# DecodeGenetics/BamQC

Measured on AMD Instinct MI355X. Metric: BAM records/sec (and GB/s vs HBM roofline), 150 bp PE, 1/2/4/8 MI355X, higher is better.
Workload: dtype u8/u32/u64 integer

## Files before the change

bamqc_amd/csrc/k_prep.hip:

```cpp
#include <algorithm>
#include <vector>
#include "kernels_common.h"
#include "prep.h"

#define PR_THREADS 256
#define PR_PER_THREAD 4
#define PR_BLOCK (PR_THREADS * PR_PER_THREAD)

__device__ __forceinline__ uint32_t wave_scan_incl_max(uint32_t v)
{
    v = max(v, (uint32_t)__builtin_amdgcn_update_dpp(0, (int)v, 0x111, 0xF, 0xF, true));
    v = max(v, (uint32_t)__builtin_amdgcn_update_dpp(0, (int)v, 0x112, 0xF, 0xF, true));
    v = max(v, (uint32_t)__builtin_amdgcn_update_dpp(0, (int)v, 0x114, 0xF, 0xF, true));
    v = max(v, (uint32_t)__builtin_amdgcn_update_dpp(0, (int)v, 0x118, 0xF, 0xF, true));
    v = max(v, (uint32_t)__builtin_amdgcn_update_dpp(0, (int)v, 0x142, 0xA, 0xF, false));
    v = max(v, (uint32_t)__builtin_amdgcn_update_dpp(0, (int)v, 0x143, 0xC, 0xF, false));
    return v;
}
__device__ __forceinline__ uint32_t block_scan_excl(uint32_t v, uint32_t* sh, uint32_t* total)
{
    const uint32_t inc = wave_scan_incl(v), w = threadIdx.x >> 6, nw = blockDim.x >> 6;
    block_sync();
    if (lane_id() == WAVE - 1) sh[w] = inc;
    block_sync();
    uint32_t base = 0, tot = 0;
    for (uint32_t k = 0; k < nw; ++k) { const uint32_t x = sh[k]; if (k < w) base += x; tot += x; }
    *total = tot;
    return base + inc - v;
}
__device__ __forceinline__ uint32_t block_scan_excl_max(uint32_t v, uint32_t* sh, uint32_t* total)
{
    const uint32_t inc = wave_scan_incl_max(v), w = threadIdx.x >> 6, nw = blockDim.x >> 6;
    block_sync();
    if (lane_id() == WAVE - 1) sh[w] = inc;
    block_sync();
    uint32_t base = 0, tot = 0;
    for (uint32_t k = 0; k < nw; ++k) { const uint32_t x = sh[k]; if (k < w) base = max(base, x); tot = max(tot, x); }
    *total = tot;
    const uint32_t prev = (uint32_t)__builtin_amdgcn_update_dpp(0, (int)inc, 0x138 , 0xF, 0xF, true);
    return max(base, prev);
}
__device__ __forceinline__ unsigned long long uniform64(unsigned long long v)
{
    return (unsigned long long)__builtin_amdgcn_readfirstlane((uint32_t)v) | (unsigned long long)__builtin_amdgcn_readfirstlane((uint32_t)(v >> 32)) << 32;
}
__device__ __forceinline__ void err_key(ErrRec* e, uint32_t read, uint32_t order)
{
    atomicMin(&e->first_key, ((unsigned long long)read << 3) | order);
}

#define PS_THREADS 1024
#define PS_PER (PR_GROUP / (PS_THREADS / 64))
__global__ __launch_bounds__(PS_THREADS) void k_prep_sizes(PrepArgs a)
{
    __shared__ unsigned long long sh[3 * PR_GROUP];
    if (blockIdx.x == 0 && threadIdx.x == 0) {
        a.err->first_key = BQC_ERRKEY_NONE; a.err->flags = 0; a.err->aux0 = a.err->aux1 = 0;
        a.desc->n_cov_extra = 0;
        if (a.pend_extra_n) *a.pend_extra_n = 0;
        if (a.replay) *a.cursor = *a.cursor_save; else *a.cursor_save = *a.cursor;
    }
    for (uint32_t k = blockIdx.x * PS_THREADS + threadIdx.x; k < a.n_sw; k += gridDim.x * PS_THREADS) a.sw_counts[k] = SwCounts{0, 0, 0, 0};
    const uint32_t nblk = (a.n + PR_BLOCK - 1) / PR_BLOCK, bg0 = blockIdx.x * PR_GROUP, nb = min((uint32_t)PR_GROUP, nblk - bg0);
    const uint32_t w = threadIdx.x >> 6, l = lane_id();
    uint4 vl[PS_PER][4];
    uint2 vc[PS_PER][4];
#pragma unroll
    for (int q = 0; q < PS_PER; ++q) {
        const uint32_t bl = w + (PS_THREADS / 64) * q;
        const unsigned long long i0 = (unsigned long long)(bg0 + bl) * PR_BLOCK;
        const bool whole = bl < nb && i0 + PR_BLOCK <= a.n;
#pragma unroll
        for (int j = 0; j < 4; ++j) {
            vl[q][j] = make_uint4(0, 0, 0, 0); vc[q][j] = make_uint2(0, 0);
            if (whole) { const uint32_t i = (uint32_t)i0 + 256u * j + 4u * l; vl[q][j] = *(const uint4*)(a.l_seq + i); vc[q][j] = *(const uint2*)(a.n_cigar + i); }
        }
    }
#pragma unroll
    for (int q = 0; q < PS_PER; ++q) {
        const uint32_t bl = w + (PS_THREADS / 64) * q;
        const unsigned long long i0 = (unsigned long long)(bg0 + bl) * PR_BLOCK;
        unsigned long long s1 = 0, s2 = 0, s3 = 0;
#pragma unroll
        for (int j = 0; j < 4; ++j) {
            const uint4 v = vl[q][j];
            s1 += (unsigned long long)((v.x + 1) / 2) + (v.y + 1) / 2 + (v.z + 1) / 2 + (v.w + 1) / 2;
            s2 += (unsigned long long)v.x + v.y + v.z + v.w;
            s3 += (vc[q][j].x & 0xFFFFu) + (vc[q][j].x >> 16) + (vc[q][j].y & 0xFFFFu) + (vc[q][j].y >> 16);
        }
        if (bl < nb && i0 + PR_BLOCK > a.n)
            for (unsigned long long i = i0 + l; i < a.n; i += WAVE) { const uint32_t L = a.l_seq[i]; s1 += (L + 1) / 2; s2 += L; s3 += a.n_cigar[i]; }
#pragma unroll
        for (int o = 32; o > 0; o >>= 1) { s1 += __shfl_xor(s1, o); s2 += __shfl_xor(s2, o); s3 += __shfl_xor(s3, o); }
        if (l == 0) { sh[3 * bl] = s1; sh[3 * bl + 1] = s2; sh[3 * bl + 2] = s3; }
    }
    block_sync();
    if (threadIdx.x < 3 * PR_GROUP) {
        const uint32_t bl = threadIdx.x / 3, k = threadIdx.x % 3;
        unsigned long long t = 0;
        for (uint32_t j = 0; j < bl; ++j) t += sh[3 * j + k];
        if (bl < nb) a.blk_sizes[3ull * (bg0 + bl) + k] = t;
        if (bl == PR_GROUP - 1) a.grp_sizes[3ull * blockIdx.x + k] = t + sh[3 * bl + k];
    }
}

struct CigarView {
    uint32_t w[4];
    const uint32_t* cg;
    __device__ __forceinline__ uint32_t at(uint32_t k) const
    {
        if (k < 4u) return k == 0u ? w[0] : k == 1u ? w[1] : k == 2u ? w[2] : w[3];
        return cg[k];
    }
};
__device__ __forceinline__ int triplet_eligible(uint32_t flag, uint32_t mapq, int32_t as, const CigarView& cv, uint32_t ncig)
{
    if (!(flag & 0x1) || !(flag & 0x2) || (flag & 0x4) || (flag & 0x8) || (flag & 0x100)) return 0;
    if (mapq < 60) return 0;
    if (as == BQC_AS_ABSENT || as < 0) return -1;
    if (as < 50) return 0;
    uint32_t clipped = 0;
    for (uint32_t k = 0; k < ncig; ++k) {
        const uint32_t wd = cv.at(k), op = wd & 15u;
        if (op == 4u || op == 5u) clipped += wd >> 4;
    }
    return clipped > 0 ? 0 : 1;
}

struct ReadIn { uint32_t L, nc, flag, lane, mapq; int32_t rid, pos, as; CovEntry ce; };
struct ReadOut { uint32_t flag, cls, tgt1; CovEntry ce; };
__device__ __forceinline__ ReadOut prep_one(const PrepArgs& a, const DevRefs& refs, uint32_t i, const ReadIn& in, uint32_t co, bool offsets_ok,
                                            const CigarView& cv, bool ref_loaded , int32_t target_in )
{
    ReadOut o;
    uint32_t flag = in.flag & (0x0FFFu | BQC_FLAG_MATE_MAIN | BQC_FLAG_NO_QUAL);
    const uint32_t L = in.L, lane = in.lane;
    uint32_t nc = in.nc;
    o.tgt1 = 0;
    if (L > a.max_read_len) err_key(a.err, i, 1);
    else if (lane >= a.n_lanes) err_key(a.err, i, 2);
    if (!offsets_ok) nc = 0;
    const bool fast = !a.no_fast && L <= BQC_FAST_MAXLEN;
    uint32_t nseg = 0;
    CovEntry ce = in.ce;
    if (!(flag & 0x900u)) {
        const bool dup = flag & 0x400u, qcf = flag & 0x200u;
        if (!dup && !qcf) {
            const int e = triplet_eligible(flag, in.mapq, in.as, cv, nc);
            if (e < 0) err_key(a.err, i, 4);
            if (e > 0) {
                const int32_t target = target_in;
                if (target < 0 || !ref_loaded) err_key(a.err, i, 5);
                else { o.tgt1 = (uint32_t)target + 1u; flag |= BQC_FLAG_TRIPLET; }
            }
        }
        if (!(flag & 0xC0u)) err_key(a.err, i, 6);
    }
    if (ce.win != BQC_COV_NONE) {
        flag |= BQC_FLAG_COV;
        const bool rc = flag & 0x10u;
        const bool pending = ce.win == BQC_COV_PENDING;
        const uint32_t pend_idx = ce.off_len;
        const int64_t pos = pending ? 0 : (int64_t)ce.off_len;
        uint32_t cc = 0;
        int64_t run_a = -1, run_z = -1;
        bool first = true;
        ce.off_len = 0;
        auto emit = [&](int64_t lo, int64_t hi) {
            if (pending) {
                if (lo < 0 || lo >= 2 * BQC_VSIZE || lo >= hi) return;
                const uint32_t len = (uint32_t)(hi - lo < 2 * BQC_VSIZE ? hi - lo : 2 * BQC_VSIZE);
                if (first) { a.pend[pend_idx] = PendRun{(uint32_t)lo, len}; first = false; return; }
                const uint32_t k = atomicAdd(a.pend_extra_n, 1u);
                if (k < a.pend_extra_cap) a.pend_extra[k] = PendExtra{pend_idx, (uint32_t)lo, len, 0};
                else atomicOr(&a.err->flags, BQC_DEVERR_INTERNAL);
                return;
            }
            hi = hi < 2 * BQC_VSIZE ? hi : 2 * BQC_VSIZE;
            if (lo < 0 || lo >= hi) return;
            const uint32_t v = (uint32_t)lo | ((uint32_t)(hi - lo) << 16);
            if (first) { ce.off_len = v; first = false; return; }
            const uint32_t k = atomicAdd(&a.desc->n_cov_extra, 1u);
            if (k < a.cov_extra_cap) a.cov_extra[k] = CovExtra{ce.win, v, lane, 0};
            else atomicOr(&a.err->flags, BQC_DEVERR_INTERNAL);
        };
        if (nc == 1u) {
            const uint32_t w = cv.w[0], op = w & 15u, nn = w >> 4;
            if (op == 0u || op == 2u) emit(pos, pos + nn);
        } else {
            for (uint32_t k = 0; k < nc; ++k) {
                const uint32_t w = cv.at(rc ? nc - 1 - k : k), op = w & 15u, nn = w >> 4;
                if (op == 4u) cc += nn;
                if (op == 0u || op == 2u) {
                    const int64_t lo = pos + (int64_t)cc, hi = lo + nn;
                    if (run_z == lo) run_z = hi;
                    else { if (run_a >= 0) emit(run_a, run_z); run_a = lo; run_z = hi; }
                    cc += nn;
                }
            }
            if (run_a >= 0) emit(run_a, run_z);
        }
        if (pending) { if (first) a.pend[pend_idx] = PendRun{0, 0}; ce = CovEntry{BQC_COV_NONE, 0}; }
    } else ce.off_len = 0;
    if (fast && (flag & BQC_FLAG_TRIPLET) && nc > 1 && L >= 3) {
        const uint32_t n0 = cv.w[0] >> 4;
        if (n0 != 0) {
            uint64_t rp = n0;
            int64_t cpos = (int64_t)in.pos + n0;
            for (uint32_t k2 = 1; k2 < nc && rp < L; ++k2) {
                const uint32_t wk = cv.at(k2), op = wk & 15u, nn = wk >> 4;
                if (op == 2u || op == 3u || op == 5u || op == 6u) cpos += nn;
                else if (op == 4u || op == 1u) rp += nn;
                else {
                    const uint64_t ia = rp > 1 ? rp : 1, ib = rp + nn < (uint64_t)L - 1 ? rp + nn : (uint64_t)L - 1;
                    const int64_t posv = cpos - (int64_t)rp;
                    if (ia < ib && posv > INT32_MIN / 2 && posv < INT32_MAX / 2) {
                        a.segs[co + nseg] = TripSeg{i, (int32_t)posv, (uint32_t)ia | ((uint32_t)ib << 8), 0};
                        ++nseg;
                    }
                    rp += nn; cpos += nn;
                }
            }
        }
    }
    o.flag = flag;
    o.ce = ce;
    o.cls = ((fast ? ((flag & 0x40u) ? 0u : 1u) : 2u) << 8) | nseg;
    return o;
}

#ifndef PR_WAVES_PER_EU
#define PR_WAVES_PER_EU 4
#endif
__global__ __launch_bounds__(PR_THREADS) __attribute__((amdgpu_waves_per_eu(PR_WAVES_PER_EU, PR_WAVES_PER_EU))) void k_prep_reads(PrepArgs a, DevRefs refs)
{
    __shared__ uint32_t sh[2 * (PR_THREADS / 64)];
    __shared__ uint32_t red[8];
    __shared__ unsigned long long gsum[3 * (PR_THREADS / 64) + 6];
    const uint32_t i0 = blockIdx.x * PR_BLOCK + 4u * threadIdx.x;
    if (threadIdx.x < 8) red[threadIdx.x] = threadIdx.x == 0 ? 0xFFFFFFFFu : 0u;
    const uint32_t grp = blockIdx.x / PR_GROUP, nblk = gridDim.x;
    unsigned long long grp_before[3] = {0, 0, 0}, grp_more[3] = {0, 0, 0}, in_grp = 0;
    for (uint32_t g = threadIdx.x + 2 * PR_THREADS; g < grp; g += PR_THREADS) {
        const unsigned long long* p = (const unsigned long long*)((const char*)a.grp_sizes + 24u * g);
        for (int k = 0; k < 3; ++k) grp_before[k] += p[k];
    }
    if (threadIdx.x < grp) {
        const unsigned long long* p = (const unsigned long long*)((const char*)a.grp_sizes + 24u * threadIdx.x);
        for (int k = 0; k < 3; ++k) grp_before[k] += p[k];
    }
    if (threadIdx.x + PR_THREADS < grp) {
        const unsigned long long* p = (const unsigned long long*)((const char*)a.grp_sizes + 24u * (threadIdx.x + PR_THREADS));
        for (int k = 0; k < 3; ++k) grp_more[k] = p[k];
    }
    if (threadIdx.x < 6) {
        const bool grp_last = (blockIdx.x + 1) % PR_GROUP == 0 || blockIdx.x + 1 == nblk;
        const unsigned long long* incl_p = grp_last ? a.grp_sizes + 3ull * grp : a.blk_sizes + 3ull * (blockIdx.x + 1);
        in_grp = threadIdx.x < 3 ? a.blk_sizes[3ull * blockIdx.x + threadIdx.x] : incl_p[threadIdx.x - 3];
    }
    auto sum_groups = [&] {
        for (int k = 0; k < 3; ++k) grp_before[k] += grp_more[k];
#pragma unroll
        for (int o = 32; o > 0; o >>= 1)
            for (int k = 0; k < 3; ++k) grp_before[k] += __shfl_xor(grp_before[k], o);
        if (lane_id() == 0) for (int k = 0; k < 3; ++k) gsum[3 * (threadIdx.x >> 6) + k] = grp_before[k];
        if (threadIdx.x < 6) gsum[3 * (PR_THREADS / 64) + threadIdx.x] = in_grp;
    };
    ReadIn in[4];
    const uint32_t nlive = i0 >= a.n ? 0u : min(4u, a.n - i0);
    if ((unsigned long long)(blockIdx.x + 1) * PR_BLOCK <= a.n) {
        const uint4 vl = *(const uint4*)(a.l_seq + i0);
        const uint2 vc = *(const uint2*)(a.n_cigar + i0), vf = *(const uint2*)(a.flag_in + i0);
        const uint32_t vlane = *(const uint32_t*)(a.lane + i0), vmq = *(const uint32_t*)(a.mapq + i0);
        const int4 vr = *(const int4*)(a.rid + i0), vp = *(const int4*)(a.pos + i0), va = *(const int4*)(a.as_ + i0);
        const uint4 c01 = *(const uint4*)(a.cov_in + i0), c23 = *(const uint4*)(a.cov_in + i0 + 2);
        asm volatile("" : "+v"(grp_before[0]), "+v"(grp_before[1]), "+v"(grp_before[2]));
        sum_groups();
        const uint32_t Ls[4] = {vl.x, vl.y, vl.z, vl.w}, ncs[4] = {vc.x & 0xFFFFu, vc.x >> 16, vc.y & 0xFFFFu, vc.y >> 16};
        const uint32_t fs[4] = {vf.x & 0xFFFFu, vf.x >> 16, vf.y & 0xFFFFu, vf.y >> 16};
        const int32_t rs[4] = {vr.x, vr.y, vr.z, vr.w}, ps[4] = {vp.x, vp.y, vp.z, vp.w}, as[4] = {va.x, va.y, va.z, va.w};
        const CovEntry cs[4] = {{c01.x, c01.y}, {c01.z, c01.w}, {c23.x, c23.y}, {c23.z, c23.w}};
#pragma unroll
        for (int j = 0; j < 4; ++j) in[j] = ReadIn{Ls[j], ncs[j], fs[j], (vlane >> (8 * j)) & 0xFFu, (vmq >> (8 * j)) & 0xFFu, rs[j], ps[j], as[j], cs[j]};
    } else {
        sum_groups();
#pragma unroll
        for (int j = 0; j < 4; ++j) {
            in[j] = ReadIn{0, 0, 0x900u, 0, 0, -1, 0, 0, CovEntry{BQC_COV_NONE, 0}};
            if ((uint32_t)j < nlive) { const uint32_t i = i0 + j; in[j] = ReadIn{a.l_seq[i], a.n_cigar[i], a.flag_in[i], a.lane[i], a.mapq[i], a.rid[i], a.pos[i], a.as_[i], a.cov_in[i]}; }
        }
    }
    uint32_t ls[4], lq[4], lc[4], ts = 0, tq = 0, tc = 0;
#pragma unroll
    for (int j = 0; j < 4; ++j) { ls[j] = ts; lq[j] = tq; lc[j] = tc; ts += (in[j].L + 1) / 2; tq += in[j].L; tc += in[j].nc; }
    uint32_t tot;
    const uint32_t xs = block_scan_excl(ts, sh, &tot), xq = block_scan_excl(tq, sh, &tot), xc = block_scan_excl(tc, sh, &tot);
    unsigned long long excl[3], incl[3];
    for (int k = 0; k < 3; ++k) {
        unsigned long long t = 0;
        for (uint32_t w = 0; w < PR_THREADS / 64; ++w) t += gsum[3 * w + k];
        grp_before[k] = uniform64(t); excl[k] = uniform64(gsum[3 * (PR_THREADS / 64) + k]); incl[k] = uniform64(gsum[3 * (PR_THREADS / 64) + 3 + k]);
    }
    unsigned long long base[3];
    if (prep_block_bases(grp_before, excl, incl, base) && threadIdx.x == 0) err_key(a.err, blockIdx.x * PR_BLOCK, 3);
    const unsigned long long bs = base[0] + xs, bq = base[1] + xq, bc = base[2] + xc;
    ReadOut out[4];
    CigarView cv[4];
    bool ref_loaded[4];
    int32_t target[4];
    unsigned long long cos[4];
    bool oks[4];
#pragma unroll
    for (int j = 0; j < 4; ++j) {
        const unsigned long long so = bs + ls[j], qo = bq + lq[j], co = bc + lc[j];
        cos[j] = co;
        oks[j] = so + (in[j].L + 1) / 2 <= 0xFFFFFFFFull && qo + in[j].L <= 0xFFFFFFFFull && co + in[j].nc <= 0xFFFFFFFFull;
        const bool live = (uint32_t)j < nlive && oks[j];
        cv[j].cg = a.cigar + (uint32_t)co;
#pragma unroll
        for (uint32_t k = 0; k < 4u; ++k) cv[j].w[k] = live && k < in[j].nc ? cv[j].cg[k] : 0u;
        const int32_t rid = in[j].rid;
        const bool rid_ok = (uint32_t)j < nlive && rid >= 0 && (uint32_t)rid < refs.n_refs;
        ref_loaded[j] = rid_ok && refs.ref[rid] != nullptr;
        target[j] = rid_ok ? (a.fasta_index ? a.fasta_index[rid] : rid) : -1;
    }
    uint32_t tmax = 0, tmin = 0xFFFFFFFFu, maxfast = 0, maxlong = 0, cnt[4] = {0, 0, 0, 0};
    bool local_bad[4] = {false, false, false, false};
#pragma unroll
    for (int j = 0; j < 4; ++j) {
        out[j] = ReadOut{0x900u, 2u << 8, 0, CovEntry{BQC_COV_NONE, 0}};
        if ((uint32_t)j >= nlive) continue;
        out[j] = prep_one(a, refs, i0 + j, in[j], (uint32_t)cos[j], oks[j], cv[j], ref_loaded[j], target[j]);
        if (out[j].tgt1) { local_bad[j] = out[j].tgt1 < tmax; tmax = max(tmax, out[j].tgt1); tmin = min(tmin, out[j].tgt1); }
        const uint32_t cl = out[j].cls >> 8;
        if (cl == 2u) maxlong = max(maxlong, in[j].L); else maxfast = max(maxfast, in[j].L);
        cnt[cl] += 1; cnt[3] += out[j].cls & 0xFFu;
    }
    if (nlive == 4u) {
        *(uint4*)(a.seq_off + i0) = make_uint4((uint32_t)bs + ls[0], (uint32_t)bs + ls[1], (uint32_t)bs + ls[2], (uint32_t)bs + ls[3]);
        *(uint4*)(a.qual_off + i0) = make_uint4((uint32_t)bq + lq[0], (uint32_t)bq + lq[1], (uint32_t)bq + lq[2], (uint32_t)bq + lq[3]);
        *(uint4*)(a.cigar_off + i0) = make_uint4((uint32_t)bc + lc[0], (uint32_t)bc + lc[1], (uint32_t)bc + lc[2], (uint32_t)bc + lc[3]);
        *(uint2*)(a.flag_out + i0) = make_uint2(out[0].flag | (out[1].flag << 16), out[2].flag | (out[3].flag << 16));
        *(uint2*)(a.cls + i0) = make_uint2(out[0].cls | (out[1].cls << 16), out[2].cls | (out[3].cls << 16));
        *(uint4*)(a.cov_out + i0) = make_uint4(out[0].ce.win, out[0].ce.off_len, out[1].ce.win, out[1].ce.off_len);
        *(uint4*)(a.cov_out + i0 + 2) = make_uint4(out[2].ce.win, out[2].ce.off_len, out[3].ce.win, out[3].ce.off_len);
    } else {
        for (uint32_t j = 0; j < nlive; ++j) {
            const uint32_t i = i0 + j;
            a.seq_off[i] = (uint32_t)bs + ls[j]; a.qual_off[i] = (uint32_t)bq + lq[j]; a.cigar_off[i] = (uint32_t)bc + lc[j];
            a.flag_out[i] = (uint16_t)out[j].flag; a.cls[i] = (uint16_t)out[j].cls; a.cov_out[i] = out[j].ce;
        }
    }
    uint32_t blk_max;
    const uint32_t before = block_scan_excl_max(tmax, sh, &blk_max);
#pragma unroll
    for (int j = 0; j < 4; ++j)
        if (out[j].tgt1 && (local_bad[j] || out[j].tgt1 < before)) err_key(a.err, i0 + j, 5);
    if (tmin != 0xFFFFFFFFu) atomicMin(&red[0], tmin);
    if (maxfast) atomicMax(&red[1], maxfast);
    if (maxlong) atomicMax(&red[2], maxlong);
    if (!a.order) {
#pragma unroll
        for (int k = 0; k < 4; ++k) { const uint32_t v = wave_sum(cnt[k]); if (lane_id() == 0 && v) atomicAdd(&red[4 + k], v); }
    }
    block_sync();
    if (threadIdx.x == 0) {
        a.blk_tgt[2ull * blockIdx.x] = blk_max;
        a.blk_tgt[2ull * blockIdx.x + 1] = red[0];
        a.blk_maxfast[2ull * blockIdx.x] = red[1];
        a.blk_maxfast[2ull * blockIdx.x + 1] = red[2];
    }
    if (!a.order && threadIdx.x < 4 && red[4 + threadIdx.x])
        atomicAdd((uint32_t*)&a.sw_counts[blockIdx.x / (BQC_SW_READS / PR_BLOCK)] + threadIdx.x, red[4 + threadIdx.x]);
}

__device__ __forceinline__ uint32_t read_class(const PrepArgs& a, uint32_t r, uint32_t* nseg)
{
    const uint32_t v = a.cls[r];
    *nseg = v & 0xFFu;
    return v >> 8;
}

__global__ __launch_bounds__(PR_THREADS) void k_build_count(PrepArgs a)
{
    __shared__ uint32_t sh[4 * (PR_THREADS / 64)];
    const SuperWindow sw = a.sws[blockIdx.x];
    uint32_t c[4] = {0, 0, 0, 0};
    for (uint32_t p = threadIdx.x; p < sw.count; p += PR_THREADS) {
        const uint32_t r = a.order ? a.order[sw.begin + p] : sw.begin + p;
        uint32_t ns;
        const uint32_t cl = read_class(a, r, &ns);
        c[cl] += 1;
        c[3] += ns;
    }
    for (int k = 0; k < 4; ++k) c[k] = wave_sum(c[k]);
    if (lane_id() == 0) for (int k = 0; k < 4; ++k) sh[4 * (threadIdx.x >> 6) + k] = c[k];
    block_sync();
    if (threadIdx.x < 4) {
        uint32_t t = 0;
        for (uint32_t w = 0; w < PR_THREADS / 64; ++w) t += sh[4 * w + threadIdx.x];
        ((uint32_t*)&a.sw_counts[blockIdx.x])[threadIdx.x] = t;
    }
}

__global__ __launch_bounds__(1024) void k_build_plan(PrepArgs a)
{
    __shared__ uint32_t sh[2 * 16 + 8];
    __shared__ uint32_t s_fast_w, s_first_bad, s_gmin;
    const uint32_t nblk = (a.n + PR_BLOCK - 1) / PR_BLOCK;
    {
        uint32_t carry = (uint32_t)(*a.cursor + 1);
        uint32_t mf = 0, gmin = 0xFFFFFFFFu;
        if (threadIdx.x == 0) { s_first_bad = 0xFFFFFFFFu; s_gmin = 0xFFFFFFFFu; }
        for (uint32_t b0 = 0; b0 < nblk; b0 += blockDim.x) {
            const uint32_t b = b0 + threadIdx.x;
            const uint32_t mx = b < nblk ? a.blk_tgt[2ull * b] : 0u, mn = b < nblk ? a.blk_tgt[2ull * b + 1] : 0xFFFFFFFFu;
            if (b < nblk) mf = max(mf, a.blk_maxfast[2ull * b]);
            uint32_t tot;
            const uint32_t before = max(carry, block_scan_excl_max(mx, sh, &tot));
            gmin = min(gmin, mn);
            if (mn < before) atomicMin(&s_first_bad, b);
            carry = max(carry, tot);
        }
        if (gmin != 0xFFFFFFFFu) atomicMin(&s_gmin, gmin);
        block_sync();
        const uint32_t bad = s_first_bad;
        if (bad != 0xFFFFFFFFu) {
            uint32_t before = (uint32_t)(*a.cursor + 1);
            for (uint32_t b = threadIdx.x; b < bad; b += blockDim.x) before = max(before, a.blk_tgt[2ull * b]);
            uint32_t tot;
            (void)block_scan_excl_max(before, sh, &tot);
            for (uint32_t i = bad * PR_BLOCK + threadIdx.x; i < min(a.n, (bad + 1) * PR_BLOCK); i += blockDim.x)
                if (a.flag_out[i] & BQC_FLAG_TRIPLET) {
                    const int32_t rid = a.rid[i];
                    const uint32_t t1 = (uint32_t)(a.fasta_index ? a.fasta_index[rid] : rid) + 1u;
                    if (t1 < tot) err_key(a.err, i, 5);
                }
        }
        for (int o = 32; o > 0; o >>= 1) mf = max(mf, (uint32_t)__shfl_xor((int)mf, o));
        block_sync();
        if (lane_id() == 0) sh[threadIdx.x >> 6] = mf;
        block_sync();
        if (threadIdx.x == 0) {
            uint32_t m = 0;
            for (uint32_t w = 0; w < blockDim.x / 64; ++w) m = max(m, sh[w]);
            s_fast_w = max(1u, (m + 8 * BQC_FAST_NH - 1) / (8 * BQC_FAST_NH));
            *a.cursor = (int32_t)carry - 1;
            if (a.cursor[1] < 0 && s_gmin != 0xFFFFFFFFu) a.cursor[1] = (int32_t)s_gmin - 1;
        }
        block_sync();
    }
    const uint32_t fast_w = s_fast_w, rpw = 64u / fast_w, h0 = (rpw + 1) / 2, h1 = rpw / 2;
    const uint32_t groups_cap = BQC_FAST_WAVES * (64u / rpw);
    const uint32_t seg_cap = groups_cap * rpw;
    uint32_t run_g = 0, run_q = 0, run_s = 0;
    for (uint32_t s0 = 0; s0 < a.n_sw; s0 += blockDim.x) {
        const uint32_t s = s0 + threadIdx.x;
        uint32_t g = 0, q = 0, sl = 0;
        if (s < a.n_sw) {
            const SwCounts c = a.sw_counts[s];
            g = max((c.n0 + h0 - 1) / h0, (c.n1 + h1 - 1) / h1);
            q = c.n_seg; sl = c.n_slow;
        }
        uint32_t tg, tq, ts;
        const uint32_t eg = run_g + block_scan_excl(g, sh, &tg), eq = run_q + block_scan_excl(q, sh, &tq), es = run_s + block_scan_excl(sl, sh, &ts);
        if (s < a.n_sw) a.sw_plan[s] = SwPlan{eg, g, eq, es};
        run_g += tg; run_q += tq; run_s += ts;
    }
    __threadfence_block();
    block_sync();
    __shared__ uint32_t s_pb, s_cf, s_cs, s_g0, s_q0, s_s0, s_ng, s_nq, s_ns, s_lane, s_sw0, s_sw1, s_longest;
    if (threadIdx.x == 0) { s_pb = 0; s_cf = 0; s_cs = 0; }
    block_sync();
    for (uint32_t st = 0; st < a.n_stretch; ++st) {
        if (threadIdx.x == 0) {
            const Stretch S = a.stretches[st];
            const SwPlan p0 = a.sw_plan[S.sw_begin];
            const SwPlan pl = a.sw_plan[S.sw_end - 1];
            const SwCounts cl = a.sw_counts[S.sw_end - 1];
            s_g0 = p0.group_base; s_q0 = p0.seg_base; s_s0 = p0.slow_base;
            s_ng = pl.group_base + pl.n_groups - p0.group_base;
            s_nq = pl.seg_base + cl.n_seg - p0.seg_base;
            s_ns = pl.slow_base + cl.n_slow - p0.slow_base;
            s_lane = S.lane; s_sw0 = S.sw_begin; s_sw1 = S.sw_end;
        }
        block_sync();
        const uint32_t pb = s_pb, ng = s_ng, nq = s_nq, ns = s_ns, lane = s_lane;
        const uint32_t nq_pad = (nq + rpw - 1) / rpw * rpw;
        const uint32_t seg0 = pb + ng * rpw, slow0 = seg0 + nq_pad;
        for (uint32_t s = s_sw0 + threadIdx.x; s < s_sw1; s += blockDim.x) {
            SwPlan p = a.sw_plan[s];
            p.group_base = pb + (p.group_base - s_g0) * rpw;
            p.seg_base = seg0 + (p.seg_base - s_q0);
            p.slow_base = slow0 + (p.slow_base - s_s0);
            a.sw_plan[s] = p;
        }
        for (uint32_t k = nq + threadIdx.x; k < nq_pad; k += blockDim.x) a.perm[seg0 + k] = 0xFFFFFFFFu;
        const uint32_t n_rc = (ng + groups_cap - 1) / groups_cap, n_sc = (nq_pad + seg_cap - 1) / seg_cap, n_lc = (ns + BQC_CHUNK_READS - 1) / BQC_CHUNK_READS;
        const uint32_t cf = s_cf, cs = s_cs;
        for (uint32_t k = threadIdx.x; k < n_rc; k += blockDim.x) {
            const uint32_t g = min(groups_cap, ng - k * groups_cap);
            if (cf + k < a.chunks_fast_cap) a.chunks_fast[cf + k] = Chunk{pb + k * groups_cap * rpw, g * rpw, lane, g * rpw, 0, 0, 0, 0};
        }
        for (uint32_t k = threadIdx.x; k < n_sc; k += blockDim.x) {
            const uint32_t e = min(seg_cap, nq_pad - k * seg_cap);
            if (cf + n_rc + k < a.chunks_fast_cap) a.chunks_fast[cf + n_rc + k] = Chunk{seg0 + k * seg_cap, e, lane, 0, 0, 0, 0, 0};
        }
        for (uint32_t k = threadIdx.x; k < n_lc; k += blockDim.x) {
            const uint32_t e = min((uint32_t)BQC_CHUNK_READS, ns - k * BQC_CHUNK_READS);
            if (cs + k < a.chunks_slow_cap) a.chunks_slow[cs + k] = Chunk{slow0 + k * BQC_CHUNK_READS, e, lane, 0, 0, 0, 0, 0};
        }
        block_sync();
        if (threadIdx.x == 0) { s_pb = slow0 + ns; s_cf = cf + n_rc + n_sc; s_cs = cs + n_lc; }
        block_sync();
    }
    uint32_t longest = 0;
    for (uint32_t b = threadIdx.x; b < nblk; b += blockDim.x) longest = max(longest, a.blk_maxfast[2ull * b + 1]);
    for (int o = 32; o > 0; o >>= 1) longest = max(longest, (uint32_t)__shfl_xor((int)longest, o));
    if (threadIdx.x == 0) s_longest = 0;
    block_sync();
    if (lane_id() == 0) atomicMax(&s_longest, longest);
    block_sync();
    if (threadIdx.x == 0) {
        if (s_pb > a.perm_cap || s_cf > a.chunks_fast_cap || s_cs > a.chunks_slow_cap) atomicOr(&a.err->flags, BQC_DEVERR_INTERNAL);
        const bool fatal = a.err->first_key != BQC_ERRKEY_NONE || (a.err->flags & BQC_DEVERR_INTERNAL);
        a.desc->fatal = fatal ? 1u : 0u;
        a.desc->n_chunks_fast = fatal ? 0u : min(s_cf, a.chunks_fast_cap);
        a.desc->n_chunks_slow = fatal ? 0u : min(s_cs, a.chunks_slow_cap);
        a.desc->fast_w = fast_w;
        a.desc->n_perm = s_pb;
        a.desc->long_max_len = s_longest;
        if (a.desc->n_cov_extra > a.cov_extra_cap) a.desc->n_cov_extra = a.cov_extra_cap;
        const unsigned long long key = a.err->first_key;
        if (key != BQC_ERRKEY_NONE) {
            const uint32_t i = (uint32_t)(key >> 3), order = (uint32_t)key & 7u;
            if (i < a.n) { a.err->aux0 = order == 1 ? a.l_seq[i] : order == 2 ? a.lane[i] : (uint32_t)a.rid[i]; a.err->aux1 = a.lane[i]; }
        }
    }
}

__device__ __forceinline__ void block_scan_excl4(uint32_t v[4], uint32_t* sh, uint32_t tot[4])
{
    const uint32_t w = threadIdx.x >> 6, nw = blockDim.x >> 6;
    uint32_t inc[4];
#pragma unroll
    for (int k = 0; k < 4; ++k) inc[k] = wave_scan_incl(v[k]);
    block_sync();
    if (lane_id() == WAVE - 1) {
#pragma unroll
        for (int k = 0; k < 4; ++k) sh[4 * w + k] = inc[k];
    }
    block_sync();
#pragma unroll
    for (int k = 0; k < 4; ++k) {
        uint32_t base = 0, t = 0;
        for (uint32_t q = 0; q < nw; ++q) { const uint32_t x = sh[4 * q + k]; if (q < w) base += x; t += x; }
        tot[k] = t;
        v[k] = base + inc[k] - v[k];
    }
}

#define SC_PER (BQC_SW_READS / PR_THREADS)
#define SC_ENT (3 * BQC_SW_READS + 128)
__global__ __launch_bounds__(PR_THREADS) void k_build_scatter(PrepArgs a)
{
    __shared__ uint32_t ent[SC_ENT];
    __shared__ uint32_t sh[4 * (PR_THREADS / 64)];
    const SuperWindow sw = a.sws[blockIdx.x];
    const SwPlan pl = a.sw_plan[blockIdx.x];
    const uint32_t fast_w = a.desc->fast_w, rpw = 64u / fast_w, h0 = (rpw + 1) / 2, h1 = rpw / 2;
    const uint32_t n_ent = pl.n_groups * rpw;
    if (n_ent > SC_ENT) { if (threadIdx.x == 0) atomicOr(&a.err->flags, BQC_DEVERR_INTERNAL); return; }
    for (uint32_t k = threadIdx.x; k < n_ent; k += PR_THREADS) ent[k] = 0xFFFFFFFFu;
    uint32_t r[SC_PER], v[SC_PER];
    const uint32_t p0 = SC_PER * threadIdx.x;
    if (!a.order && p0 + SC_PER <= sw.count && ((sw.begin + p0) & 7u) == 0u) {
        const uint4 x = *(const uint4*)(a.cls + sw.begin + p0), y = *(const uint4*)(a.cls + sw.begin + p0 + 8);
        const uint32_t wd[8] = {x.x, x.y, x.z, x.w, y.x, y.y, y.z, y.w};
#pragma unroll
        for (int k = 0; k < SC_PER; ++k) { r[k] = sw.begin + p0 + k; v[k] = (wd[k >> 1] >> (16 * (k & 1))) & 0xFFFFu; }
    } else {
#pragma unroll
        for (int k = 0; k < SC_PER; ++k) { const uint32_t p = p0 + k; r[k] = p < sw.count ? (a.order ? a.order[sw.begin + p] : sw.begin + p) : 0xFFFFFFFFu; }
#pragma unroll
        for (int k = 0; k < SC_PER; ++k) v[k] = r[k] != 0xFFFFFFFFu ? a.cls[r[k]] : 3u << 8;
    }
    uint32_t c[4] = {0, 0, 0, 0};
#pragma unroll
    for (int k = 0; k < SC_PER; ++k) {
        const uint32_t cl = v[k] >> 8;
        c[0] += cl == 0u; c[1] += cl == 1u; c[2] += cl == 2u; c[3] += cl < 3u ? v[k] & 0xFFu : 0u;
    }
    uint32_t co[SC_PER];
#pragma unroll
    for (int k = 0; k < SC_PER; ++k) co[k] = (v[k] >> 8) < 3u && (v[k] & 0xFFu) ? a.cigar_off[r[k]] : 0u;
    uint32_t tot[4];
    block_scan_excl4(c, sh, tot);
    uint32_t k0 = c[0], k1 = c[1], k2 = c[2], k3 = c[3];
#pragma unroll
    for (int k = 0; k < SC_PER; ++k) {
        const uint32_t cl = v[k] >> 8, ns = v[k] & 0xFFu;
        if (cl == 0u) { ent[(k0 / h0) * rpw + k0 % h0] = r[k]; ++k0; }
        else if (cl == 1u) { ent[(k1 / h1) * rpw + h0 + k1 % h1] = r[k]; ++k1; }
        else if (cl == 2u) a.perm[pl.slow_base + k2++] = r[k];
        if (cl < 3u && ns) { for (uint32_t j = 0; j < ns; ++j) a.perm[pl.seg_base + k3 + j] = BQC_ENTRY_SEG | (co[k] + j); k3 += ns; }
    }
    block_sync();
    for (uint32_t k = threadIdx.x; k < n_ent; k += PR_THREADS) a.perm[pl.group_base + k] = ent[k];
}

extern "C" void bqc_launch_prep(const PrepArgs& a, const DevRefs& refs, hipStream_t s, hipEvent_t after_reads)
{
    if (a.n == 0) return;
    const uint32_t nblk = (a.n + PR_BLOCK - 1) / PR_BLOCK;
    hipLaunchKernelGGL(k_prep_sizes, dim3((nblk + PR_GROUP - 1) / PR_GROUP), dim3(PS_THREADS), 0, s, a);
    hipLaunchKernelGGL(k_prep_reads, dim3(nblk), dim3(PR_THREADS), 0, s, a, refs);
    if (after_reads) (void)hipEventRecord(after_reads, s);
    if (a.order) hipLaunchKernelGGL(k_build_count, dim3(a.n_sw), dim3(PR_THREADS), 0, s, a);
    hipLaunchKernelGGL(k_build_plan, dim3(1), dim3(1024), 0, s, a);
    hipLaunchKernelGGL(k_build_scatter, dim3(a.n_sw), dim3(PR_THREADS), 0, s, a);
}

extern "C" uint32_t bqc_prep_group(void) { return PR_GROUP; }
extern "C" uint32_t bqc_prep_bases(const uint64_t* blk_totals, uint32_t n_blocks, uint64_t* bases)
{
    const uint32_t n_groups = (n_blocks + PR_GROUP - 1) / PR_GROUP;
    std::vector<unsigned long long> blk(3ull * n_blocks), grp(3ull * n_groups);
    for (uint32_t g = 0; g < n_groups; ++g)
        for (int k = 0; k < 3; ++k) {
            unsigned long long t = 0;
            for (uint32_t b = g * PR_GROUP; b < std::min(n_blocks, (g + 1) * PR_GROUP); ++b) { blk[3ull * b + k] = t; t += blk_totals[3ull * b + k]; }
            grp[3ull * g + k] = t;
        }
    uint32_t first_bad = 0xFFFFFFFFu;
    for (uint32_t b = 0; b < n_blocks; ++b) {
        const uint32_t g = b / PR_GROUP;
        const bool grp_last = (b + 1) % PR_GROUP == 0 || b + 1 == n_blocks;
        const unsigned long long* incl = grp_last ? &grp[3ull * g] : &blk[3ull * (b + 1)];
        unsigned long long before[3] = {0, 0, 0}, base[3];
        for (uint32_t g2 = 0; g2 < g; ++g2)
            for (int k = 0; k < 3; ++k) before[k] += grp[3ull * g2 + k];
        if (prep_block_bases(before, &blk[3ull * b], incl, base)) first_bad = std::min(first_bad, b);
        for (int k = 0; k < 3; ++k) bases[3ull * b + k] = base[k];
    }
    return first_bad;
}

__device__ __forceinline__ uint32_t pend_interval(uint32_t pos, uint32_t c0, uint32_t len)
{
    const uint32_t lo = pos + c0;
    if (!len || lo >= 2u * BQC_VSIZE) return 0u;
    const uint32_t hi = min(lo + len, 2u * BQC_VSIZE);
    return lo | ((hi - lo) << 16);
}
__global__ __launch_bounds__(256) void k_pend_cov(uint32_t n, const CovEntry* __restrict__ cov_in, const PendRun* __restrict__ pend, const PendExtra* __restrict__ extra,
                                                     const uint32_t* __restrict__ extra_n, uint32_t extra_cap, const uint8_t* __restrict__ lane,
                                                     CovEntry* __restrict__ cov_out, CovExtra* __restrict__ cov_extra, BatchDesc* __restrict__ desc)
{
    const uint32_t ne = min(*extra_n, extra_cap);
    for (uint32_t i = blockIdx.x * blockDim.x + threadIdx.x; i < n; i += gridDim.x * blockDim.x) {
        const CovEntry ce = cov_in[i];
        const PendRun r = pend[i];
        cov_out[i] = CovEntry{ce.win, pend_interval(ce.off_len, r.c0, r.len)};
    }
    for (uint32_t e = blockIdx.x * blockDim.x + threadIdx.x; e < ne; e += gridDim.x * blockDim.x) {
        const PendExtra x = extra[e];
        const CovEntry ce = cov_in[x.idx];
        cov_extra[e] = CovExtra{ce.win, pend_interval(ce.off_len, x.c0, x.len), lane[x.idx], 0};
    }
    if (blockIdx.x == 0 && threadIdx.x == 0) { desc->n_cov_extra = ne; desc->fatal = 0; }
}
extern "C" void bqc_launch_pend_cov(uint32_t n, const CovEntry* cov_in, const PendRun* pend, const PendExtra* extra, const uint32_t* extra_n, uint32_t extra_cap,
                                    const uint8_t* lane, CovEntry* cov_out, CovExtra* cov_extra, BatchDesc* desc, hipStream_t s)
{
    if (!n) return;
    hipLaunchKernelGGL(k_pend_cov, dim3(std::min<uint32_t>((n + 255) / 256, 4096u)), dim3(256), 0, s, n, cov_in, pend, extra, extra_n, extra_cap, lane, cov_out, cov_extra, desc);
}
```

bamqc_amd/csrc/prep.h:

```cpp
#pragma once
#include <hip/hip_runtime.h>
#include <stdint.h>
#include "device_types.h"

#ifndef PR_GROUP
#define PR_GROUP 32
#endif
static_assert(PR_GROUP >= 16 && (PR_GROUP & (PR_GROUP - 1)) == 0, "PR_GROUP: a power of two, 16 or more");

__host__ __device__ inline bool prep_block_bases(const unsigned long long before[3], const unsigned long long excl[3], const unsigned long long incl[3],
                                                 unsigned long long base[3])
{
    bool over = false;
    for (int k = 0; k < 3; ++k) {
        base[k] = before[k] + excl[k];
        over |= before[k] + incl[k] > 0xFFFFFFFFull;
    }
    return over;
}

struct Stretch {
    uint32_t lane, sw_begin, sw_end, pad;
};

struct PrepArgs {
    uint32_t n;
    uint32_t n_lanes, max_read_len;
    uint32_t no_fast;
    uint32_t replay;
    const uint16_t* flag_in;
    const uint8_t* mapq;
    const uint8_t* lane;
    const int32_t* rid;
    const int32_t* pos;
    const int32_t* as_;
    const uint32_t* l_seq;
    const uint16_t* n_cigar;
    const uint8_t* qual;
    const uint32_t* cigar;
    const CovEntry* cov_in;
    const uint32_t* order;
    const SuperWindow* sws;
    uint32_t n_sw;
    const Stretch* stretches;
    uint32_t n_stretch;
    const int32_t* fasta_index;
    uint16_t* flag_out;
    uint32_t* seq_off;
    uint32_t* qual_off;
    uint32_t* cigar_off;
    CovEntry* cov_out;
    CovExtra* cov_extra;
    uint32_t cov_extra_cap;
    PendRun* pend;
    PendExtra* pend_extra;
    uint32_t* pend_extra_n;
    uint32_t pend_extra_cap;
    uint16_t* cls;
    TripSeg* segs;
    uint32_t* perm;
    uint32_t perm_cap;
    Chunk* chunks_fast;
    uint32_t chunks_fast_cap;
    Chunk* chunks_slow;
    uint32_t chunks_slow_cap;
    BatchDesc* desc;
    ErrRec* err;
    int32_t* cursor;
    int32_t* cursor_save;
    unsigned long long* blk_sizes;
    unsigned long long* grp_sizes;
    uint32_t* blk_tgt;
    uint32_t* blk_maxfast;
    SwCounts* sw_counts;
    SwPlan* sw_plan;
};

extern "C" void bqc_launch_prep(const PrepArgs& a, const DevRefs& refs, hipStream_t s, hipEvent_t after_reads);
extern "C" uint32_t bqc_prep_bases(const uint64_t* blk_totals, uint32_t n_blocks, uint64_t* bases);
extern "C" uint32_t bqc_prep_group(void);
extern "C" void bqc_launch_pend_cov(uint32_t n, const CovEntry* cov_in, const PendRun* pend, const PendExtra* extra, const uint32_t* extra_n, uint32_t extra_cap,
                                    const uint8_t* lane, CovEntry* cov_out, CovExtra* cov_extra, BatchDesc* desc, hipStream_t s);
```

Measured before the change: 4.547 billion.

## Interleave not-ready fast reads evenly across wave groups in scatter

Tags fast reads that can take the full triplet path with a READY bit in the class word. The scatter kernel then spreads the not-ready reads evenly over the wave groups using magic-number division, rather than packing reads by rank. The aim is to balance per-wave work and cut divergence from slow-path reads piling into the same waves. A host helper mirrors the mapping for testing, and the change adds per-entry integer arithmetic in the scatter step.

```diff
diff --git a/bamqc_amd/csrc/k_prep.hip b/bamqc_amd/csrc/k_prep.hip
--- a/bamqc_amd/csrc/k_prep.hip
+++ b/bamqc_amd/csrc/k_prep.hip
@@ -226,6 +226,7 @@
     o.flag = flag;
     o.ce = ce;
     o.cls = ((fast ? ((flag & 0x40u) ? 0u : 1u) : 2u) << 8) | nseg;
+    if (fast && (flag & BQC_FLAG_TRIPLET) && L >= 3 && nc >= 1 && !(flag & BQC_FLAG_NO_QUAL)) o.cls |= PREP_CLS_READY;
     return o;
 }
 
@@ -332,7 +333,7 @@
         if ((uint32_t)j >= nlive) continue;
         out[j] = prep_one(a, refs, i0 + j, in[j], (uint32_t)cos[j], oks[j], cv[j], ref_loaded[j], target[j]);
         if (out[j].tgt1) { local_bad[j] = out[j].tgt1 < tmax; tmax = max(tmax, out[j].tgt1); tmin = min(tmin, out[j].tgt1); }
-        const uint32_t cl = out[j].cls >> 8;
+        const uint32_t cl = PREP_CLS_CLASS(out[j].cls);
         if (cl == 2u) maxlong = max(maxlong, in[j].L); else maxfast = max(maxfast, in[j].L);
         cnt[cl] += 1; cnt[3] += out[j].cls & 0xFFu;
     }
@@ -378,7 +379,7 @@
 {
     const uint32_t v = a.cls[r];
     *nseg = v & 0xFFu;
-    return v >> 8;
+    return PREP_CLS_CLASS(v);
 }
 
 __global__ __launch_bounds__(PR_THREADS) void k_build_count(PrepArgs a)
@@ -568,7 +569,7 @@
     __shared__ uint32_t sh[4 * (PR_THREADS / 64)];
     const SuperWindow sw = a.sws[blockIdx.x];
     const SwPlan pl = a.sw_plan[blockIdx.x];
-    const uint32_t fast_w = a.desc->fast_w, rpw = 64u / fast_w, h0 = (rpw + 1) / 2, h1 = rpw / 2;
+    const uint32_t fast_w = a.desc->fast_w, rpw = 64u / fast_w;
     const uint32_t n_ent = pl.n_groups * rpw;
     if (n_ent > SC_ENT) { if (threadIdx.x == 0) atomicOr(&a.err->flags, BQC_DEVERR_INTERNAL); return; }
     for (uint32_t k = threadIdx.x; k < n_ent; k += PR_THREADS) ent[k] = 0xFFFFFFFFu;
@@ -588,20 +589,32 @@
     uint32_t c[4] = {0, 0, 0, 0};
 #pragma unroll
     for (int k = 0; k < SC_PER; ++k) {
-        const uint32_t cl = v[k] >> 8;
-        c[0] += cl == 0u; c[1] += cl == 1u; c[2] += cl == 2u; c[3] += cl < 3u ? v[k] & 0xFFu : 0u;
+        const uint32_t cl = PREP_CLS_CLASS(v[k]), one = (v[k] & PREP_CLS_READY) ? 1u : 0x10000u;
+        c[0] += cl == 0u ? one : 0u; c[1] += cl == 1u ? one : 0u; c[2] += cl == 2u; c[3] += cl < 3u ? v[k] & 0xFFu : 0u;
     }
     uint32_t co[SC_PER];
 #pragma unroll
-    for (int k = 0; k < SC_PER; ++k) co[k] = (v[k] >> 8) < 3u && (v[k] & 0xFFu) ? a.cigar_off[r[k]] : 0u;
+    for (int k = 0; k < SC_PER; ++k) co[k] = PREP_CLS_CLASS(v[k]) < 3u && (v[k] & 0xFFu) ? a.cigar_off[r[k]] : 0u;
     uint32_t tot[4];
     block_scan_excl4(c, sh, tot);
     uint32_t k0 = c[0], k1 = c[1], k2 = c[2], k3 = c[3];
+    if (!(tot[0] | tot[1])) {
+#pragma unroll
+        for (int k = 0; k < SC_PER; ++k)
+            if (PREP_CLS_CLASS(v[k]) == 2u) a.perm[pl.slow_base + k2++] = r[k];
+        return;
+    }
+    const PrepSlotMap M = prep_slot_map(rpw, pl.n_groups, tot[0] >> 16, tot[1] >> 16);
 #pragma unroll
     for (int k = 0; k < SC_PER; ++k) {
-        const uint32_t cl = v[k] >> 8, ns = v[k] & 0xFFu;
-        if (cl == 0u) { ent[(k0 / h0) * rpw + k0 % h0] = r[k]; ++k0; }
-        else if (cl == 1u) { ent[(k1 / h1) * rpw + h0 + k1 % h1] = r[k]; ++k1; }
+        const uint32_t cl = PREP_CLS_CLASS(v[k]), ns = v[k] & 0xFFu;
+        if (cl < 2u) {
+            const bool rdy = v[k] & PREP_CLS_READY;
+            const uint32_t e = prep_slot_entry(M, cl, rdy, cl ? k1 : k0);
+            if (e < n_ent) ent[e] = r[k];
+            const uint32_t one = rdy ? 1u : 0x10000u;
+            k0 += cl ? 0u : one; k1 += cl ? one : 0u;
+        }
         else if (cl == 2u) a.perm[pl.slow_base + k2++] = r[k];
         if (cl < 3u && ns) { for (uint32_t j = 0; j < ns; ++j) a.perm[pl.seg_base + k3 + j] = BQC_ENTRY_SEG | (co[k] + j); k3 += ns; }
     }
@@ -622,6 +635,24 @@
 }
 
 extern "C" uint32_t bqc_prep_group(void) { return PR_GROUP; }
+extern "C" void bqc_prep_slot_map(uint32_t rpw, uint32_t n_cases, const uint32_t* begin, const uint8_t* kind, uint32_t* entry, uint32_t* groups)
+{
+    const uint32_t h0 = (rpw + 1) / 2, h1 = rpw / 2;
+    for (uint32_t cs = 0; cs < n_cases; ++cs) {
+        uint32_t tot[2] = {0, 0}, c[2] = {0, 0};
+        for (uint32_t p = begin[cs]; p < begin[cs + 1]; ++p) tot[kind[p] & 1u] += (kind[p] & 2u) ? 1u : 0x10000u;
+        const uint32_t n0 = (tot[0] & 0xFFFFu) + (tot[0] >> 16), n1 = (tot[1] & 0xFFFFu) + (tot[1] >> 16);
+        const uint32_t G = std::max((n0 + h0 - 1) / h0, h1 ? (n1 + h1 - 1) / h1 : 0u);
+        const PrepSlotMap M = prep_slot_map(rpw, G, tot[0] >> 16, tot[1] >> 16);
+        groups[2 * cs] = G; groups[2 * cs + 1] = M.I;
+        for (uint32_t p = begin[cs]; p < begin[cs + 1]; ++p) {
+            const uint32_t mate = kind[p] & 1u;
+            const bool rdy = kind[p] & 2u;
+            entry[p] = prep_slot_entry(M, mate, rdy, c[mate]);
+            c[mate] += rdy ? 1u : 0x10000u;
+        }
+    }
+}
 extern "C" uint32_t bqc_prep_bases(const uint64_t* blk_totals, uint32_t n_blocks, uint64_t* bases)
 {
     const uint32_t n_groups = (n_blocks + PR_GROUP - 1) / PR_GROUP;
diff --git a/bamqc_amd/csrc/prep.h b/bamqc_amd/csrc/prep.h
--- a/bamqc_amd/csrc/prep.h
+++ b/bamqc_amd/csrc/prep.h
@@ -17,6 +17,40 @@
         over |= before[k] + incl[k] > 0xFFFFFFFFull;
     }
     return over;
+}
+
+#define PREP_CLS_CLASS(v) (((v) >> 8) & 3u)
+#define PREP_CLS_READY 0x400u
+
+static_assert(BQC_SW_READS <= 32768, "prep_slot_entry: ranks of a super-window in 16 bits, (G + 1) G + I + G < 2^31");
+struct PrepSlotMap { uint32_t rpw, G, I, D, h0, h1, m_h0, m_h1, m_I, m_D; };
+__host__ __device__ inline uint32_t prep_magic(uint32_t d) { return 0xFFFFFFFFu / d + (d > 1u ? 1u : 0u); }
+__host__ __device__ inline uint32_t prep_div(uint32_t n, uint32_t d, uint32_t m )
+{
+    const uint32_t q = (uint32_t)(((unsigned long long)n * m) >> 32);
+    const int32_t r = (int32_t)(n - q * d);
+    return q + (r >= (int32_t)d ? 1u : 0u) - (r < 0 ? 1u : 0u);
+}
+__host__ __device__ inline PrepSlotMap prep_slot_map(uint32_t rpw, uint32_t G, uint32_t i0, uint32_t i1)
+{
+    PrepSlotMap M;
+    M.rpw = rpw; M.G = G; M.h0 = (rpw + 1) / 2; M.h1 = rpw / 2;
+    const uint32_t f0 = i0 / M.h0, f1 = M.h1 ? i1 / M.h1 : 0u;
+    M.I = f0 < f1 ? f0 : f1;
+    if (M.I > G) M.I = G;
+    M.D = G - M.I;
+    M.m_h0 = prep_magic(M.h0); M.m_h1 = prep_magic(M.h1 ? M.h1 : 1u); M.m_I = prep_magic(M.I ? M.I : 1u); M.m_D = prep_magic(M.D ? M.D : 1u);
+    return M;
+}
+__host__ __device__ inline uint32_t prep_slot_entry(const PrepSlotMap& M, uint32_t mate, bool ready, uint32_t ranks)
+{
+    const uint32_t n_ready = ranks & 0xFFFFu, n_other = ranks >> 16;
+    const uint32_t h = mate ? M.h1 : M.h0, m_h = mate ? M.m_h1 : M.m_h0, first = mate ? M.h0 : 0u, aside = h * M.I;
+    const bool set_aside = !ready && n_other < aside;
+    const uint32_t k = set_aside ? n_other : n_ready + (n_other > aside ? n_other - aside : 0u);
+    const uint32_t q = prep_div(k, h, m_h);
+    const uint32_t g = prep_div(set_aside ? (q + 1u) * M.G + M.I - 1u : q * M.G, set_aside ? M.I : M.D ? M.D : 1u, set_aside ? M.m_I : M.m_D) - (set_aside ? 1u : 0u);
+    return g * M.rpw + first + (k - q * h);
 }
 
 struct Stretch {
@@ -79,5 +113,6 @@
 extern "C" void bqc_launch_prep(const PrepArgs& a, const DevRefs& refs, hipStream_t s, hipEvent_t after_reads);
 extern "C" uint32_t bqc_prep_bases(const uint64_t* blk_totals, uint32_t n_blocks, uint64_t* bases);
 extern "C" uint32_t bqc_prep_group(void);
+extern "C" void bqc_prep_slot_map(uint32_t rpw, uint32_t n_cases, const uint32_t* begin, const uint8_t* kind, uint32_t* entry, uint32_t* groups);
 extern "C" void bqc_launch_pend_cov(uint32_t n, const CovEntry* cov_in, const PendRun* pend, const PendExtra* extra, const uint32_t* extra_n, uint32_t extra_cap,
                                     const uint8_t* lane, CovEntry* cov_out, CovExtra* cov_extra, BatchDesc* desc, hipStream_t s);
```

Result: faster. 4.622 billion (median of 6 runs) (+1.6%).
